# YoshikiMaekawa2000/ccv_mppi_path_tracker

Hardware: AMD Instinct MI355X
Metric: trajectory rollouts/s (K×iters/s) + ms/MPPI-iteration, diff-drive T=50 (higher is better)
Workload: dtype f64; 1 GPU; C2: diff_drive K=65536 T=50 sinusoid, u_dim=2, launch parameters; samples_per_gpu=65536, horizon=50, state_store=True

## Files before the change

ccv_mppi_path_tracker_amd/csrc/mppi_epilogue.h:

```cpp
#pragma once
#include "mppi_device_util.h"
#include "mppi_kernels.h"
#include "mppi_produce.h"

namespace ccv {

constexpr int kUpdRB = 15;
constexpr int kUpdCH = 4 * kUpdRB;

template <int BR_, int NW_>
struct UpdRowsT {
    static constexpr int BR = BR_, NW = NW_;
    int R, wv;
    __device__ __forceinline__ int count() const {
        int n = 0;
        for (int r0 = wv * BR; r0 < R; r0 += NW * BR) n += min(BR, R - r0);
        return n;
    }
    __device__ __forceinline__ int row(const int m) const { return ((m / BR) * NW + wv) * BR + m % BR; }
};

template <int MODE>
using UpdT = std::conditional_t<MODE == MODE_FUSED, float, double>;
template <class T, class ROWS>
__device__ __forceinline__ void pc_update_fetch(const RolloutArgs& A, T (&v)[kUpdCH], const ROWS& rows, const int m0,
                                                const int mcount, const int kk) {
    const size_t pitch = (size_t)A.pitch;
#pragma unroll
    for (int i = 0; i < kUpdCH; ++i) {
        const size_t at = (size_t)rows.row(min(m0 + i, mcount - 1)) * pitch + kk;
        if constexpr (std::is_same<T, float>::value) v[i] = A.z[at];
        else v[i] = A.u[at];
    }
}

template <int RB, int MODEL, bool LOOP = false, class SH, class T, class ROWS>
__device__ __forceinline__ void pc_reduce_rows(const RolloutArgs& A, const SH& sh, double* buf, T (&v)[kUpdCH], const ROWS& rows,
                                               const int mcount, const double wgt, const int lane, const int kk,
                                               const bool fast_clamp = false) {
    static_assert(RB <= 16 && kUpdCH % RB == 0, "batch size");
    constexpr int STRIDE = kPcSamples + 2;
    const int rr = lane >> 2, q = lane & 3;
    const int col_w = lane + (lane >> 5), col_r = q * 16 + (q >> 1);
    auto batch = [&](auto V0_, const int base) {
        constexpr int V0 = decltype(V0_)::value;
        const int nrows = min(RB, mcount - base);
        double nomv[RB];
        if constexpr (std::is_same<T, float>::value) {
#pragma unroll
            for (int r = 0; r < RB; ++r) nomv[r] = sh.nom[rows.row(min(base + r, mcount - 1))];
        }
        auto products = [&](auto FAST_) {
            constexpr bool FAST = decltype(FAST_)::value;
            static_for<RB>([&](auto RR) {
                constexpr int r = decltype(RR)::value;
                if constexpr (std::is_same<T, float>::value) {
                    constexpr int UD = udim_of(MODEL);
                    static_assert(ROWS::BR % UD == 0 && kUpdCH % UD == 0 && (!LOOP || RB % UD == 0), "row dealing vs control dimension");
                    constexpr int d = (V0 + r) % UD;
                    buf[r * STRIDE + col_w] = wgt * pc_control_from_normal_at<MODEL, d, FAST>(A, v[V0 + r], nomv[r]);
                } else {
                    buf[r * STRIDE + col_w] = wgt * v[V0 + r];
                }
            });
        };
        if (std::is_same<T, float>::value && fast_clamp) products(std::true_type{});
        else products(std::false_type{});
        __builtin_amdgcn_s_waitcnt(0xC07F);
        __builtin_amdgcn_wave_barrier();
        double acc = 0.0;
        if (rr < nrows) {
#pragma unroll
            for (int i = 0; i < 16; ++i) acc += buf[rr * STRIDE + col_r + i];
        }
        acc += dpp_move<kDppXor1>(acc);
        acc += dpp_move<kDppXor2>(acc);
        if (rr < nrows && q == 0) A.partial[(size_t)rows.row(base + rr) * A.nparts + blockIdx.x] = acc;
        __builtin_amdgcn_wave_barrier();
    };
    for (int chunk0 = 0; chunk0 < mcount; chunk0 += kUpdCH) {
        if (chunk0 != 0) pc_update_fetch(A, v, rows, chunk0, mcount, kk);
        if constexpr (LOOP) {
#pragma clang loop unroll(disable)
            for (int base = chunk0; base < min(mcount, chunk0 + kUpdCH); base += RB) {
                batch(std::integral_constant<int, 0>{}, base);
#pragma unroll
                for (int i = 0; i + RB < kUpdCH; ++i) v[i] = v[i + RB];
            }
        } else {
            static_for<kUpdCH / RB>([&](auto BB) {
                constexpr int bb = decltype(BB)::value;
                if (chunk0 + bb * RB < mcount) batch(std::integral_constant<int, bb * RB>{}, chunk0 + bb * RB);
            });
        }
    }
}

__device__ __forceinline__ void pc_block_stats(const RolloutArgs& A, const int R, const double wgt, const double total, const bool live,
                                               const int lane) {
    const double sw = wave_sum(wgt);
    const double mn = wave_min(live ? total : INFINITY);
    const double mx = wave_max(live ? total : -INFINITY);
    const double nz = wave_sum((live && wgt == 0.0) ? 1.0 : 0.0);
    if (lane == 0) {
        A.partial[(size_t)R * A.nparts + blockIdx.x] = sw;
        A.statpart[blockIdx.x * 3 + 0] = mn;
        A.statpart[blockIdx.x * 3 + 1] = mx;
        A.statpart[blockIdx.x * 3 + 2] = nz;
    }
}

__device__ __forceinline__ double pc_shifted_weight(const RolloutArgs& A, const double total, const bool live) {
    const double mg = wave_min(live ? total : INFINITY);
    const double shift = mg < INFINITY ? mg : 0.0;
    return live ? exp(-(total - shift) / A.lambda) : 0.0;
}
template <bool SHIFT>
__device__ __forceinline__ double pc_weight(const RolloutArgs& A, const double total, const bool live) {
    if constexpr (SHIFT) return pc_shifted_weight(A, total, live);
    else return live ? exp(-total / A.lambda) : 0.0;
}

}
```

ccv_mppi_path_tracker_amd/csrc/mppi_rollout_r4.h:

```cpp
#pragma once
#include "mppi_consume.h"
#include "mppi_epilogue.h"
#include "mppi_handoff.h"
#include "mppi_produce.h"

namespace ccv {

constexpr int kR4Waves = 4;
template <int MODEL>
constexpr int kR4RB = MODEL == CCV_MPPI_FULL_BODY ? 15 : 12;

struct R4Rows {
    static constexpr int BR = 60;
    int first, n;
    __device__ __forceinline__ int count() const { return n; }
    __device__ __forceinline__ int row(const int m) const { return first + m; }
};
template <int UD>
__device__ __forceinline__ R4Rows r4_rows(const int H, const int nblocks, const int wv, int& nb_early) {
    const int R = (H - 1) * UD;
    nb_early = max(0, nblocks - 3);
    if (nb_early == 0) {
        const int per = ((R / UD + kR4Waves - 1) / kR4Waves) * UD;
        const int first = min(R, wv * per);
        return R4Rows{first, min(per, R - first)};
    }
    const int r_early = min(R, nb_early * kTU * UD);
    const int half_e = ((r_early / UD + 1) / 2) * UD, half_l = (((R - r_early) / UD + 1) / 2) * UD;
    switch (wv) {
        case 0: return R4Rows{0, half_e};
        case 1: return R4Rows{half_e, r_early - half_e};
        case 2: return R4Rows{r_early, half_l};
        default: return R4Rows{r_early + half_l, R - r_early - half_l};
    }
}
template <class T>
__device__ __forceinline__ void r4_fetch0(const RolloutArgs& A, T (&v)[kUpdCH], const R4Rows& rows, const int kk) {
    const size_t pitch = (size_t)A.pitch;
    const char* p0;
    if constexpr (std::is_same<T, float>::value) p0 = reinterpret_cast<const char*>(A.z + (size_t)rows.first * pitch);
    else p0 = reinterpret_cast<const char*>(A.u + (size_t)rows.first * pitch);
    const uint32_t koff = (uint32_t)kk * (uint32_t)sizeof(T);
#pragma unroll
    for (int i = 0; i < kUpdCH; ++i) {
        v[i] = 0;
        if (i < rows.n) v[i] = *reinterpret_cast<const T*>(p0 + (size_t)i * (pitch * sizeof(T)) + koff);
    }
}

template <int MODEL>
struct R4Shared {
    static constexpr bool kStage = true;
    static constexpr int kPBuf = 2;
    double p[2][kTU][2][kPcSamples];
    double2 ab[kMaxH + 4];
    double c[kMaxH + 4];
    float zs[2][kTU * udim_of(MODEL)][kPcSamples];
    double cost[kR4Waves][kPcSamples];
    alignas(32) double nom[(kMaxH + 8) * udim_of(MODEL)];
    int seq[8];
    int nan_seen[kR4Waves];
};

template <int MODEL, class SH>
__device__ __forceinline__ void r4_noise_block(const RolloutArgs& A, SH& sh, const int b, const int lane, const uint32_t kg) {
    pc_for_call_groups<MODEL>([&](auto C0_, auto CN_) {
        constexpr int C0 = decltype(C0_)::value, CN = decltype(CN_)::value;
        float z[4 * CN];
        pc_block_normals<MODEL, C0, CN>(A, b, kg, z);
#pragma unroll
        for (int i = 0; i < 4 * CN; ++i) sh.zs[b & 1][4 * C0 + i][lane] = z[i];
    });
}

template <int MODEL, class SH>
__device__ __forceinline__ void r4_noise_call(const RolloutArgs& A, SH& sh, const int b, const int call, const int lane, const uint32_t kg) {
    constexpr int UD = udim_of(MODEL);
    const Philox4 r = philox4x32_10(kg, (uint32_t)((b * kTU * UD) >> 2) + (uint32_t)call, A.iter_lo, A.iter_hi, A.seed_lo, A.seed_hi);
    float z[4];
    box_muller_f32(r.x, r.y, z[0], z[1]);
    box_muller_f32(r.z, r.w, z[2], z[3]);
#pragma unroll
    for (int i = 0; i < 4; ++i) sh.zs[b & 1][4 * call + i][lane] = z[i];
}

template <int MODEL, int NT>
struct R4Staged {
    static constexpr int kPerThread = ((kMaxH - 1 + kTU) * udim_of(MODEL) + NT - 1) / NT;
    double wa, wb, wc;
    double nv[kPerThread];
    double S;
};
template <int MODEL, int NT, bool BATCH = false>
__device__ __forceinline__ void r4_stage_issue(const RolloutArgs& A, const Window& Wk, const int tid, R4Staged<MODEL, NT>& L) {
    static_assert(NT >= kMaxH + 4, "one window point per thread");
    const int H = A.H, R = (H - 1) * udim_of(MODEL);
    L.wa = L.wb = 0.0;
    L.wc = INFINITY;
    if (tid < H) {
        if constexpr (BATCH) {
            const double* win = reinterpret_cast<const double*>(A.frame) + kBatchHeadDoubles;
            L.wa = win[tid];
            L.wb = win[H + tid];
            L.wc = win[2 * H + tid];
        } else if (A.frame) {
            const Window& W = A.frame->W;
            L.wa = W.a[tid];
            L.wb = W.b[tid];
            L.wc = W.c[tid];
        } else {
            L.wa = Wk.a[tid];
            L.wb = Wk.b[tid];
            L.wc = Wk.c[tid];
        }
    }
    const double* src = A.pending_vec ? A.pending_vec + 1 : A.nominal;
    L.S = A.pending_vec ? A.pending_vec[0] : 1.0;
#pragma unroll
    for (int i = 0; i < R4Staged<MODEL, NT>::kPerThread; ++i) {
        const int j = tid + i * NT;
        L.nv[i] = j < R ? src[j] : 0.0;
    }
}
template <int MODEL, int NT, class SH>
__device__ __forceinline__ bool r4_stage_commit(const RolloutArgs& A, SH& sh, const int tid, const R4Staged<MODEL, NT>& L) {
    const int H = A.H, H4 = (H + 3) & ~3, R = (H - 1) * udim_of(MODEL);
    if (tid < H4) {
        sh.ab[tid] = make_double2(L.wa, L.wb);
        sh.c[tid] = L.wc;
    }
    bool bad = false;
#pragma unroll
    for (int i = 0; i < R4Staged<MODEL, NT>::kPerThread; ++i) {
        const int j = tid + i * NT;
        if (j < R + kTU * udim_of(MODEL)) {
            const double v = (A.pending_vec && j < R) ? L.nv[i] / L.S : L.nv[i];
            sh.nom[j] = v;
            bad |= v != v;
            if (blockIdx.x == 0 && j < R) {
                if (A.pending_vec) A.nominal_w[j] = v;
                A.nominal_used[j] = v;
            }
        }
    }
    if (A.pending_vec && blockIdx.x == 0 && tid == 0) A.stats_w[0] = L.S;
    return bad;
}

struct R4Lane {
    int lane, k, kk;
    bool live;
    uint32_t kg;
};
__device__ __forceinline__ R4Lane r4_lane(const RolloutArgs& A) {
    R4Lane L;
    L.lane = (int)__builtin_amdgcn_mbcnt_hi(~0u, __builtin_amdgcn_mbcnt_lo(~0u, 0u));
    asm volatile("" : "+v"(L.lane));
    L.k = (int)blockIdx.x * kPcSamples + L.lane;
    L.live = L.k < A.K;
    L.kk = L.live ? L.k : A.K - 1;
    L.kg = (uint32_t)(A.k_offset + L.kk);
    return L;
}

template <int MODEL, int MODE, bool WIDE = false, bool TAIL = false, BatchForm FORM = BatchForm::Single, bool SHIFT = false>
__global__ __launch_bounds__(kR4Waves * 64, MODEL == CCV_MPPI_FULL_BODY ? 1 : 4) void k_rollout_r4(const RolloutArgs Ak, const Window Wk) {
    constexpr bool BATCH = FORM >= BatchForm::Batch, VARIED = FORM >= BatchForm::Varied, OBST = FORM >= BatchForm::Obst,
                   MOVING = FORM >= BatchForm::Moving, GRID = FORM >= BatchForm::Grid;
    constexpr bool FB = MODEL == CCV_MPPI_FULL_BODY;
    constexpr bool COST = MODE != MODE_ROLLOUT;
    constexpr int UD = udim_of(MODEL);
    static_assert(!WIDE || (MODEL == CCV_MPPI_DIFF_DRIVE && MODE == MODE_FUSED), "the wide-turn form exists for the fused diff-drive iteration");
    static_assert(!TAIL || MODE == MODE_FUSED, "the stage-wise modes carry the masked producer anyway");
    static_assert(!BATCH || MODE == MODE_FUSED, "batch handles run the fused iteration only");
    static_assert(!SHIFT || VARIED, "the shifted weights are built on the per-instance-parameter kernels");
    static_assert(!OBST || MODE == MODE_FUSED, "the obstacle term is the fused iteration's");
    __shared__ R4Shared<MODEL> sh;
    ObstLds* obst_lds = nullptr;
    ObstMovLds* obst_mov = nullptr;
    if constexpr (MOVING) {
        __shared__ ObstMovLds s_obst_mov;
        obst_mov = &s_obst_mov;
    } else if constexpr (OBST) {
        __shared__ ObstLds s_obst;
        obst_lds = &s_obst;
    }
    static_assert(offsetof(R4Shared<MODEL>, zs) + sizeof(sh.zs) >= kR4Waves * kR4RB<MODEL> * (kPcSamples + 2) * sizeof(double), "epilogue buffers");
    touch_rollout_args();
    const RolloutArgs A = rollout_view<MODEL, BATCH, VARIED>(Ak);
    if (A.prio_rotate) pc_set_priority((int)blockIdx.x / A.cu_count);
    const int H = A.H;
    const int wv = __builtin_amdgcn_readfirstlane(threadIdx.x >> 6);
    if (wv == 0) CCV_DIAG_STAMP(A, 0);
    const int nblocks = (H + kTU - 1) / kTU;
    const int nstates = FB ? H - 2 : H;
    const int nfull = MODE == MODE_FUSED ? (TAIL ? (H - 1 + kTU - kPartialMin) / kTU : (H - 1) / kTU) : 0;
    int* const seq_noise = &sh.seq[0];
    if (threadIdx.x < 8) sh.seq[threadIdx.x] = (threadIdx.x == 0 && nfull > 0) ? 1 : 0;
    PcState<MODEL> S;
    bool bad_nominal = false;
    if constexpr (MODE == MODE_FUSED) {
        R4Staged<MODEL, kR4Waves * 64> staged;
        r4_stage_issue<MODEL, kR4Waves * 64, BATCH>(A, Wk, (int)threadIdx.x, staged);
        if (nfull > 0) {
            constexpr int NCALL = kTU * UD / 4;
            const R4Lane L = r4_lane(A);
            for (int c = wv; c < NCALL; c += kR4Waves) r4_noise_call<MODEL>(A, sh, 0, c, L.lane, L.kg);
        }
        if (wv == 0) CCV_DIAG_STAMP(A, 3);
        if (wv == 1) {
            pc_initial_state<MODEL>(A, S);
            CCV_DIAG_STAMP(A, 1);
        }
        bad_nominal = r4_stage_commit<MODEL>(A, sh, (int)threadIdx.x, staged);
        if constexpr (OBST) {
            const int j = (int)threadIdx.x - 2 * 64;
            if (j >= 0 && j < kMaxObst) obst_stage_form<FORM>(A, obst_lds, obst_mov, j);
        }
        const bool wave_bad = __builtin_amdgcn_ballot_w64(bad_nominal) != 0ull;
        if (r4_lane(A).lane == 0) sh.nan_seen[wv] = wave_bad ? 1 : 0;
    } else {
        if constexpr (COST) stage_window(A, Wk, sh, kR4Waves * 64);
        if (wv == 1) pc_initial_state<MODEL>(A, S);
    }
    __syncthreads();
    if (wv == 1) CCV_DIAG_STAMP(A, 2);
    const bool fast_clamp = MODE == MODE_FUSED && A.fast_clamp &&
                            __builtin_amdgcn_readfirstlane(sh.nan_seen[0] | sh.nan_seen[1] | sh.nan_seen[2] | sh.nan_seen[3]) == 0;
    int* const seq_ready = &sh.seq[1];
    int* const seq_dist = &sh.seq[2];
    int* const seq_store = &sh.seq[3];
    int* const seq_stored = &sh.seq[4];
    int nb_early;
    R4Rows rows = r4_rows<UD>(H, nblocks, wv, nb_early);
    if (!(COST && A.fuse_update)) rows.n = 0;
    UpdT<MODE> upd[kUpdCH];
    auto early_fetch = [&]() {
        if constexpr (MODE == MODE_FUSED) {
            if (rows.n > 0 && nb_early > 0) {
                pc_wait_for(seq_stored, nb_early);
                r4_fetch0(A, upd, rows, r4_lane(A).kk);
            }
        }
    };
    if (wv == 0) {
        if constexpr (MODE == MODE_FUSED) {
            const R4Lane L = r4_lane(A);
            const int lane = L.lane;
            const uint32_t kg = L.kg;
            for (int b = 1; b < nfull; ++b) {
                r4_rotate_priority(A, b, 0);
                if (b >= 2) {
                    pc_wait_for(seq_ready, b - 1);
                    pc_wait_for(seq_store, b - 1);
                }
                r4_noise_block<MODEL>(A, sh, b, lane, kg);
                pc_publish(seq_noise, b + 1);
            }
            CCV_DIAG_STAMP(A, 15);
        }
        if constexpr (COST) sh.cost[0][r4_lane(A).lane] = 0.0;
        if (A.prio_rotate) __builtin_amdgcn_s_setprio(0);
        early_fetch();
    } else if (wv == 1) {
        const R4Lane L = r4_lane(A);
        const int lane = L.lane, k = L.k, kk = L.kk;
        const bool live = L.live;
        const uint32_t kg = L.kg;
        double cost = 0.0;
        cost += pc_initial_cost<MODEL, MODE>(A);
        constexpr unsigned LDSZ = kNormalsInLds | (WIDE ? kWideTurn : 0u);
        for (int b = 0; b < nblocks; ++b) {
            r4_rotate_priority(A, b, 1);
            if (b >= 2) {
                pc_wait_for(seq_dist, b - 1);
                pc_wait_for(seq_store, b - 1);
            }
            const int nctl = min(kTU, H - 1 - b * kTU);
            if (b < nfull) {
                pc_wait_for(seq_noise, b + 1);
                if (b == 0) CCV_DIAG_STAMP(A, 4);
                if (!TAIL || nctl == kTU) {
                    if (fast_clamp)
                        pc_produce_batched<MODEL, MODE, R4Shared<MODEL>, LDSZ | kFastClamp>(A, sh, S, cost, b, lane, k, kk, live, kg);
                    else
                        pc_produce_batched<MODEL, MODE, R4Shared<MODEL>, LDSZ>(A, sh, S, cost, b, lane, k, kk, live, kg);
                } else if constexpr (TAIL) {
                    if (fast_clamp && nctl == 6)
                        pc_produce_batched<MODEL, MODE, R4Shared<MODEL>, LDSZ | kPartialBlock | kFastClamp, 6>(A, sh, S, cost, b, lane, k, kk, live, kg, kNoNormalsAhead, nctl);
                    else if (fast_clamp)
                        pc_produce_batched<MODEL, MODE, R4Shared<MODEL>, LDSZ | kPartialBlock | kFastClamp>(A, sh, S, cost, b, lane, k, kk, live, kg, kNoNormalsAhead, nctl);
                    else
                        pc_produce_batched<MODEL, MODE, R4Shared<MODEL>, LDSZ | kPartialBlock>(A, sh, S, cost, b, lane, k, kk, live, kg, kNoNormalsAhead, nctl);
                }
            } else if (MODE != MODE_FUSED && nctl == kTU) {
                pc_produce_batched<MODEL, MODE>(A, sh, S, cost, b, lane, k, kk, live, kg);
            } else if (MODE != MODE_FUSED && nctl >= kPartialMin) {
                pc_produce_batched<MODEL, MODE, R4Shared<MODEL>, kPartialBlock>(A, sh, S, cost, b, lane, k, kk, live, kg, kNoNormalsAhead, nctl);
            } else {
                pc_produce<MODEL, MODE, false>(A, sh, S, cost, b, lane, k, kk, live, kg);
            }
            pc_publish(seq_ready, b + 1);
            if (b == 0) CCV_DIAG_STAMP(A, 5);
        }
        CCV_DIAG_STAMP(A, 6);
        if constexpr (COST) sh.cost[1][lane] = cost;
        if (A.prio_rotate) __builtin_amdgcn_s_setprio(0);
        early_fetch();
    } else if (wv == 2) {
        int prune_on = 1;
        const int lane = r4_lane(A).lane;
        double cost = 0.0;
        for (int b = 0; b < nblocks; ++b) {
            r4_rotate_priority(A, b, 2);
            pc_wait_for(seq_ready, b + 1);
            bool taken = false;
            if constexpr (COST) {
                const int nv = min(kConsumeStates, nstates - b * kTU);
                taken = nv > 0;
                pc_consume_states<MODEL, R4Shared<MODEL>, kLeanRegisters | consume_discs(FORM)>(nv, A, sh, cost, b, lane, &prune_on, obst_lds, obst_mov, seq_dist, b + 1);
            }
            if (!taken) pc_publish(seq_dist, b + 1);
            if (b == 0) CCV_DIAG_STAMP(A, 14);
        }
        CCV_DIAG_STAMP(A, 7);
        if constexpr (COST) sh.cost[2][lane] = cost;
    } else {
        const size_t pitch = (size_t)A.pitch;
        const R4Lane L = r4_lane(A);
        const int lane = L.lane;
        const uint32_t koff4 = (uint32_t)L.k * 4u, koff8 = (uint32_t)L.k * 8u;
        GridAcc grid_acc{};
        if constexpr (GRID) grid_acc = GridAcc{grid_row(A), 0.0, nstates, nullptr};
        for (int b = 0; b < nblocks; ++b) {
            r4_rotate_priority(A, b, 3);
            pc_wait_for(seq_ready, b + 1);
            const int t0 = b * kTU;
            float zv[kTU * UD];
            double xv[kTU], yv[kTU];
            if constexpr (MODE == MODE_FUSED) {
#pragma unroll
                for (int r = 0; r < kTU * UD; ++r) zv[r] = sh.zs[b & 1][r][lane];
            }
            if constexpr (MODE != MODE_COST) {
#pragma unroll
                for (int tt = 0; tt < kTU; ++tt) {
                    xv[tt] = sh.p[b & 1][tt][0][lane];
                    yv[tt] = sh.p[b & 1][tt][1][lane];
                }
            }
            asm volatile("s_waitcnt lgkmcnt(0)" ::: "memory");
            pc_publish(seq_store, b + 1);
            GridTap tap[kTU];
            if constexpr (GRID) {
                grid_issue(grid_acc, xv, yv, tap);
            }
            if constexpr (MODE == MODE_FUSED) {
                const int nrows = min(kTU, H - 1 - t0) * UD;
                char* const zrow = reinterpret_cast<char*>(A.z + (size_t)(t0 * UD) * pitch);
                static_for<kTU * UD>([&](auto RR) {
                    constexpr int r = decltype(RR)::value;
                    if (r < nrows) pc_store_f32(zrow + (size_t)r * (pitch * 4), koff4, zv[r]);
                });
            }
            if constexpr (MODE != MODE_COST) {
                if (A.store_xy) {
                    const int nst = min(kTU, H - t0);
                    char* const xrow = reinterpret_cast<char*>(A.xs + (size_t)t0 * pitch);
                    char* const yrow = reinterpret_cast<char*>(A.ys + (size_t)t0 * pitch);
#pragma unroll
                    for (int tt = 0; tt < kTU; ++tt) {
                        if (tt < nst) {
                            pc_store_f64_stream(xrow + (size_t)tt * (pitch * 8), koff8, xv[tt]);
                            pc_store_f64_stream(yrow + (size_t)tt * (pitch * 8), koff8, yv[tt]);
                        }
                    }
                }
            }
            if constexpr (GRID) {
                grid_sum(grid_acc, tap, t0);
            }
            if constexpr (MODE == MODE_FUSED) {
                constexpr int kRowsZ = kTU * UD, kRowsAll = kTU * UD + 2 * kTU;
                static_assert(kRowsAll <= 63, "vmcnt is a 6-bit counter");
                if (t0 + kTU <= H - 1 && A.store_xy) asm volatile("s_waitcnt vmcnt(%0)" ::"n"(kRowsAll) : "memory");
                else if (t0 + kTU <= H - 1) asm volatile("s_waitcnt vmcnt(%0)" ::"n"(kRowsZ) : "memory");
                else asm volatile("s_waitcnt vmcnt(0)" ::: "memory");
                pc_publish(seq_stored, b);
            }
        }
        asm volatile("s_waitcnt vmcnt(0)" ::: "memory");
        if constexpr (GRID) sh.cost[3][lane] = grid_acc.G;
        else if constexpr (COST) sh.cost[3][lane] = 0.0;
    }
    if (A.prio_rotate) __builtin_amdgcn_s_setprio(0);
    if constexpr (COST) {
        const int R = (H - 1) * UD;
        const int mcount = rows.n;
        const R4Lane L = r4_lane(A);
        const int lane = L.lane, k = L.k, kk = L.kk;
        const bool live = L.live;
        pc_barrier_lds();
        if (wv == 0) CCV_DIAG_STAMP(A, 8);
        bool from_lds = false;
        if constexpr (MODE == MODE_FUSED) {
            from_lds = nblocks <= 2;
            if (from_lds) {
                constexpr int kMaxLdsRows = 4 * UD;
                static_assert(kMaxLdsRows <= kUpdCH, "first chunk");
#pragma unroll
                for (int i = 0; i < kMaxLdsRows; ++i) {
                    const int row = rows.first + min(i, max(mcount - 1, 0));
                    upd[i] = sh.zs[(row / (kTU * UD)) & 1][row % (kTU * UD)][lane];
                }
                pc_barrier_lds();
            }
        }
        if (!from_lds && (MODE != MODE_FUSED || wv >= 2 || nb_early == 0) && mcount > 0) r4_fetch0(A, upd, rows, kk);
        double total_;
        if constexpr (GRID) {
            total_ = ((sh.cost[0][lane] + sh.cost[1][lane]) + sh.cost[2][lane]) + 0.0;
            const ConstGridRow g = grid_row(A);
            if (g) total_ = fma(g->w, sh.cost[3][lane], total_);
        } else {
            total_ = ((sh.cost[0][lane] + sh.cost[1][lane]) + sh.cost[2][lane]) + sh.cost[3][lane];
        }
        const double total = total_;
        double wgt_;
        if constexpr (SHIFT) wgt_ = pc_shifted_weight(A, total, live);
        else wgt_ = live ? exp(-total / A.lambda) : 0.0;
        const double wgt = wgt_;
        if (wv == 0 && live) {
            A.cost[k] = total;
            A.w[k] = wgt;
        }
        if (wv == 0) CCV_DIAG_STAMP_VALUE(A, 9, wgt);
        if (wv == 2) CCV_DIAG_STAMP_VALUE(A, 11, wgt);
        if (A.fuse_update) {
            double* buf = &sh.p[0][0][0][0] + wv * (kR4RB<MODEL> * (kPcSamples + 2));
            pc_reduce_rows<kR4RB<MODEL>, MODEL, true>(A, sh, buf, upd, rows, mcount, wgt, lane, kk, fast_clamp);
            if (wv == kR4Waves - 1) pc_block_stats(A, R, wgt, total, live, lane);
        }
        if (wv == 0) CCV_DIAG_STAMP(A, 10);
        if (wv == 2) CCV_DIAG_STAMP(A, 12);
        if (wv == 3) CCV_DIAG_STAMP(A, 13);
    }
}

}
```

Measured before the change: 1.915 billion rollouts/s.

## Hold diff-drive update chunk in indexed vector registers instead of shifting arrays

For the steering diff-drive model, the fused update epilogue now keeps its per-lane chunk of fetched control values in a LoopChunk of 16-wide vectors, indexed by batch. Previously the array was shifted down by RB after every batch. Fetches use a contiguous-row pointer walk in which the stride drops to zero past the end, and warm-start nominals are read unclamped. The aim is to remove the register-shuffle moves and address recomputation in the rolled batch loop. The cost is dynamic vector-element indexing, which may lower to index-mode moves or scratch memory.

Result: slower. 1.891 billion rollouts/s (-1.2%).

```diff
diff --git a/ccv_mppi_path_tracker_amd/csrc/mppi_epilogue.h b/ccv_mppi_path_tracker_amd/csrc/mppi_epilogue.h
--- a/ccv_mppi_path_tracker_amd/csrc/mppi_epilogue.h
+++ b/ccv_mppi_path_tracker_amd/csrc/mppi_epilogue.h
@@ -34,19 +34,86 @@
     }
 }
 
-template <int RB, int MODEL, bool LOOP = false, class SH, class T, class ROWS>
-__device__ __forceinline__ void pc_reduce_rows(const RolloutArgs& A, const SH& sh, double* buf, T (&v)[kUpdCH], const ROWS& rows,
+constexpr int kLoopBatches = 4;
+template <class T, int RB>
+struct LoopChunk {
+    static constexpr int W = sizeof(T) / 4, NV = (RB * W + 3) / 4;
+    static_assert(sizeof(T) == 4 * W && (W == 1 || W == 2) && kLoopBatches == 4, "32-bit words, four batches to a vector's row");
+    typedef uint32_t Vec __attribute__((ext_vector_type(16)));
+    typedef std::conditional_t<W == 1, uint32_t, uint64_t> Bits;
+    Vec q[NV];
+    static __device__ __forceinline__ constexpr int VI(const int s) { return s / 4; }
+    static __device__ __forceinline__ constexpr int EI(const int s, const int b) { return (s % 4) * 4 + b; }
+    template <int I>
+    __device__ __forceinline__ void set(const T x) {
+        constexpr int b = I / RB, r = I % RB;
+        static_assert(b < kLoopBatches, "chunk");
+        const Bits bits = __builtin_bit_cast(Bits, x);
+#pragma unroll
+        for (int w = 0; w < W; ++w) q[VI(r * W + w)][EI(r * W + w, b)] = (uint32_t)(bits >> (w * 32 % (8 * (int)sizeof(Bits))));
+    }
+    template <int r>
+    __device__ __forceinline__ T get(const int b) const {
+        Bits bits = 0;
+#pragma unroll
+        for (int w = 0; w < W; ++w) bits |= (Bits)q[VI(r * W + w)][EI(r * W + w, b)] << (w * 32 % (8 * (int)sizeof(Bits)));
+        return __builtin_bit_cast(T, bits);
+    }
+};
+
+template <int RB, class T>
+__device__ __forceinline__ void pc_fetch_range(const RolloutArgs& A, LoopChunk<T, RB>& v, const int first, const int n, const int kk) {
+    typedef const __attribute__((address_space(1))) char* gptr;
+    const uint32_t rowbytes = (uint32_t)A.pitch * (uint32_t)sizeof(T);
+    gptr p;
+    if constexpr (std::is_same<T, float>::value) p = (gptr)A.z;
+    else p = (gptr)A.u;
+    p += (size_t)first * rowbytes;
+    uint32_t koff = (uint32_t)kk * (uint32_t)sizeof(T);
+    static_for<kLoopBatches>([&](auto BB) {
+        constexpr int b0 = decltype(BB)::value * RB;
+        if (b0 < n) {
+            static_for<RB>([&](auto RR) {
+                constexpr int r = decltype(RR)::value;
+                asm volatile("" : "+s"(p), "+v"(koff));
+                v.template set<b0 + r>(*reinterpret_cast<const __attribute__((address_space(1))) T*>(p + koff));
+                uint32_t step = b0 + r + 1 < n ? rowbytes : 0u;
+                asm("" : "+s"(step));
+                p += step;
+            });
+        }
+    });
+}
+
+template <class V>
+struct UpdElem;
+template <class T>
+struct UpdElem<T[kUpdCH]> { using type = T; };
+template <class T, int RB>
+struct UpdElem<LoopChunk<T, RB>> { using type = T; };
+template <class V>
+constexpr bool kIsLoopChunk = !std::is_array<V>::value;
+template <int RB, int MODEL, bool LOOP = false, class SH, class V, class ROWS>
+__device__ __forceinline__ void pc_reduce_rows(const RolloutArgs& A, const SH& sh, double* buf, V& v, const ROWS& rows,
                                                const int mcount, const double wgt, const int lane, const int kk,
                                                const bool fast_clamp = false) {
+    using T = typename UpdElem<V>::type;
+    constexpr bool CHUNK = kIsLoopChunk<V>;
+    static_assert(!CHUNK || LOOP, "a LoopChunk is the LOOP form's");
     static_assert(RB <= 16 && kUpdCH % RB == 0, "batch size");
     constexpr int STRIDE = kPcSamples + 2;
     const int rr = lane >> 2, q = lane & 3;
     const int col_w = lane + (lane >> 5), col_r = q * 16 + (q >> 1);
-    auto batch = [&](auto V0_, const int base) {
+    auto batch = [&](auto V0_, const int base, auto& v) {
         constexpr int V0 = decltype(V0_)::value;
         const int nrows = min(RB, mcount - base);
         double nomv[RB];
-        if constexpr (std::is_same<T, float>::value) {
+        if constexpr (std::is_same<T, float>::value && CHUNK) {
+            static_assert(!CHUNK || RB <= kTU * udim_of(MODEL), "a batch's warm start is read unclamped");
+            const double* const nom = &sh.nom[rows.row(base)];
+#pragma unroll
+            for (int r = 0; r < RB; ++r) nomv[r] = nom[r];
+        } else if constexpr (std::is_same<T, float>::value) {
 #pragma unroll
             for (int r = 0; r < RB; ++r) nomv[r] = sh.nom[rows.row(min(base + r, mcount - 1))];
         }
@@ -78,19 +145,31 @@
         if (rr < nrows && q == 0) A.partial[(size_t)rows.row(base + rr) * A.nparts + blockIdx.x] = acc;
         __builtin_amdgcn_wave_barrier();
     };
-    for (int chunk0 = 0; chunk0 < mcount; chunk0 += kUpdCH) {
-        if (chunk0 != 0) pc_update_fetch(A, v, rows, chunk0, mcount, kk);
-        if constexpr (LOOP) {
+    constexpr int CH = CHUNK ? kLoopBatches * RB : kUpdCH;
+    for (int chunk0 = 0; chunk0 < mcount; chunk0 += CH) {
+        if constexpr (CHUNK) {
+            static_assert(!CHUNK || ROWS::kContiguous, "a chunk is one range of rows");
+            if (chunk0 != 0) pc_fetch_range<RB>(A, v, rows.row(chunk0), mcount - chunk0, kk);
+            int b = 0;
+#pragma clang loop unroll(disable)
+            for (int base = chunk0; base < min(mcount, chunk0 + CH); base += RB, ++b) {
+                T cur[RB];
+                static_for<RB>([&](auto RR) { cur[decltype(RR)::value] = v.template get<decltype(RR)::value>(b); });
+                batch(std::integral_constant<int, 0>{}, base, cur);
+            }
+        } else if constexpr (LOOP) {
+            if (chunk0 != 0) pc_update_fetch(A, v, rows, chunk0, mcount, kk);
 #pragma clang loop unroll(disable)
             for (int base = chunk0; base < min(mcount, chunk0 + kUpdCH); base += RB) {
-                batch(std::integral_constant<int, 0>{}, base);
+                batch(std::integral_constant<int, 0>{}, base, v);
 #pragma unroll
                 for (int i = 0; i + RB < kUpdCH; ++i) v[i] = v[i + RB];
             }
         } else {
+            if (chunk0 != 0) pc_update_fetch(A, v, rows, chunk0, mcount, kk);
             static_for<kUpdCH / RB>([&](auto BB) {
                 constexpr int bb = decltype(BB)::value;
-                if (chunk0 + bb * RB < mcount) batch(std::integral_constant<int, bb * RB>{}, chunk0 + bb * RB);
+                if (chunk0 + bb * RB < mcount) batch(std::integral_constant<int, bb * RB>{}, chunk0 + bb * RB, v);
             });
         }
     }
diff --git a/ccv_mppi_path_tracker_amd/csrc/mppi_rollout_r4.h b/ccv_mppi_path_tracker_amd/csrc/mppi_rollout_r4.h
--- a/ccv_mppi_path_tracker_amd/csrc/mppi_rollout_r4.h
+++ b/ccv_mppi_path_tracker_amd/csrc/mppi_rollout_r4.h
@@ -12,6 +12,7 @@
 
 struct R4Rows {
     static constexpr int BR = 60;
+    static constexpr bool kContiguous = true;
     int first, n;
     __device__ __forceinline__ int count() const { return n; }
     __device__ __forceinline__ int row(const int m) const { return first + m; }
@@ -34,7 +35,15 @@
         default: return R4Rows{r_early + half_l, R - r_early - half_l};
     }
 }
-template <class T>
+template <int MODEL>
+constexpr bool kR4Indexed = MODEL == CCV_MPPI_STEERING_DIFF_DRIVE;
+template <int MODEL, class T>
+using R4Upd = std::conditional_t<kR4Indexed<MODEL>, LoopChunk<T, kR4RB<MODEL>>, T[kUpdCH]>;
+template <int MODEL, class T>
+__device__ __forceinline__ void r4_fetch0(const RolloutArgs& A, LoopChunk<T, kR4RB<MODEL>>& v, const R4Rows& rows, const int kk) {
+    pc_fetch_range(A, v, rows.first, rows.n, kk);
+}
+template <int MODEL, class T>
 __device__ __forceinline__ void r4_fetch0(const RolloutArgs& A, T (&v)[kUpdCH], const R4Rows& rows, const int kk) {
     const size_t pitch = (size_t)A.pitch;
     const char* p0;
@@ -234,12 +243,12 @@
     int nb_early;
     R4Rows rows = r4_rows<UD>(H, nblocks, wv, nb_early);
     if (!(COST && A.fuse_update)) rows.n = 0;
-    UpdT<MODE> upd[kUpdCH];
+    R4Upd<MODEL, UpdT<MODE>> upd;
     auto early_fetch = [&]() {
         if constexpr (MODE == MODE_FUSED) {
             if (rows.n > 0 && nb_early > 0) {
                 pc_wait_for(seq_stored, nb_early);
-                r4_fetch0(A, upd, rows, r4_lane(A).kk);
+                r4_fetch0<MODEL>(A, upd, rows, r4_lane(A).kk);
             }
         }
     };
@@ -407,16 +416,24 @@
             from_lds = nblocks <= 2;
             if (from_lds) {
                 constexpr int kMaxLdsRows = 4 * UD;
-                static_assert(kMaxLdsRows <= kUpdCH, "first chunk");
-#pragma unroll
-                for (int i = 0; i < kMaxLdsRows; ++i) {
-                    const int row = rows.first + min(i, max(mcount - 1, 0));
-                    upd[i] = sh.zs[(row / (kTU * UD)) & 1][row % (kTU * UD)][lane];
+                static_assert(kMaxLdsRows <= kLoopBatches * kR4RB<MODEL> && kMaxLdsRows <= kUpdCH, "first chunk");
+                if constexpr (kR4Indexed<MODEL>) {
+                    static_for<kMaxLdsRows>([&](auto II) {
+                        constexpr int i = decltype(II)::value;
+                        const int row = rows.first + min(i, max(mcount - 1, 0));
+                        upd.template set<i>(sh.zs[(row / (kTU * UD)) & 1][row % (kTU * UD)][lane]);
+                    });
+                } else {
+#pragma unroll
+                    for (int i = 0; i < kMaxLdsRows; ++i) {
+                        const int row = rows.first + min(i, max(mcount - 1, 0));
+                        upd[i] = sh.zs[(row / (kTU * UD)) & 1][row % (kTU * UD)][lane];
+                    }
                 }
                 pc_barrier_lds();
             }
         }
-        if (!from_lds && (MODE != MODE_FUSED || wv >= 2 || nb_early == 0) && mcount > 0) r4_fetch0(A, upd, rows, kk);
+        if (!from_lds && (MODE != MODE_FUSED || wv >= 2 || nb_early == 0) && mcount > 0) r4_fetch0<MODEL>(A, upd, rows, kk);
         double total_;
         if constexpr (GRID) {
             total_ = ((sh.cost[0][lane] + sh.cost[1][lane]) + sh.cost[2][lane]) + 0.0;
```
